# bitlayer-org/tap-stark

Measured on AMD Instinct MI355X. Metric: trace cells/sec (proofs/sec alongside), 2^20x64 BabyBear trace, higher is better.
Workload: dtype u32

## Files before the change

tap-stark_amd/csrc/kernels.hpp:

```cpp
#pragma once
#include <stdint.h>

#include "bb.hpp"
#include "context.hpp"

namespace ts {

struct ColMat {
    uint32_t* d = nullptr;
    uint64_t height = 0;
    uint32_t width = 0;
    uint64_t col_stride = 0;
};

void launch_build_twiddles(Context& ctx, uint32_t* W, uint32_t* Winv, unsigned log_size);
void launch_build_shift_tables(Context& ctx, uint32_t* lo, uint32_t* hi, uint32_t n_hi,
                               uint32_t n_cosets, uint32_t shift_mont, unsigned log_N,
                               unsigned log_blowup, uint32_t scale_mont);
const uint32_t* coset_scale_table(Context& ctx, unsigned log_n, unsigned log_blowup, uint32_t shift);
void launch_transpose_bitrev(Context& ctx, const uint32_t* src, uint32_t* dst, unsigned log_n,
                             uint32_t w, uint64_t dst_col_stride, uint32_t src_width = 0);
bool launch_transpose_bitrev_r16(Context& ctx, const uint32_t* src, uint32_t* dst, unsigned log_n, uint32_t w,
                                 uint64_t dst_col_stride, uint32_t src_width = 0);
void launch_transpose_plain(Context& ctx, const uint32_t* src, uint32_t* dst, uint64_t n, uint32_t w,
                            uint64_t dst_col_stride);
void launch_transpose_to_row_major(Context& ctx, const uint32_t* src, uint64_t col_stride,
                                   uint32_t* dst, uint64_t h, uint32_t w);
void coset_lde(Context& ctx, uint32_t* evals, uint64_t in_col_stride, uint32_t ncols, unsigned log_n,
               unsigned log_blowup, uint32_t shift, uint32_t* out, uint64_t out_col_stride,
               uint32_t beta0 = 0, uint32_t n_beta = 0, bool first_round_done = false,
               uint32_t* evals2 = nullptr, uint32_t shift2 = 0, uint32_t gw = 0);

constexpr int MAX_BATCH_MATS = 64;
struct LeafMats {
    const uint32_t* d[MAX_BATCH_MATS];
    uint64_t col_stride[MAX_BATCH_MATS];
    uint32_t width[MAX_BATCH_MATS];
    uint8_t row_shift[MAX_BATCH_MATS];
    uint32_t n_mats;
    uint32_t total_width;
    const uint32_t* const* cols;
};
void launch_leaf_hash(Context& ctx, const LeafMats& mats, uint64_t height, uint32_t* digests);
void launch_leaf_hash_ef_pairs(Context& ctx, const uint32_t* vec, uint64_t n_rows, uint32_t* digests);
struct DevChallenger;
bool launch_merkle_levels(Context& ctx, uint32_t* tree, unsigned log_leaves,
                          DevChallenger* ch = nullptr, uint32_t* root_out = nullptr,
                          Ef* beta_out = nullptr);
bool leaf_tree_enabled(unsigned log_leaves);
bool launch_commit_tree(Context& ctx, const LeafMats& mats, unsigned log_leaves, uint32_t* tree,
                        DevChallenger* ch = nullptr, uint32_t* root_out = nullptr, Ef* beta_out = nullptr);
bool launch_commit_tree_ef_pairs(Context& ctx, const uint32_t* vec, unsigned log_leaves, uint32_t* tree,
                                 DevChallenger* ch = nullptr, uint32_t* root_out = nullptr,
                                 Ef* beta_out = nullptr);
void launch_shard_top(Context& ctx, const uint32_t* subroots, uint32_t G, uint32_t* top,
                      DevChallenger* ch, uint32_t* root_out, Ef* beta_out);
void launch_merkle_one_level(Context& ctx, const uint32_t* children, uint32_t* parents,
                             uint64_t n_parents);
void launch_merkle_inject(Context& ctx, uint32_t* nodes, const uint32_t* inj, uint64_t n);
inline uint64_t merkle_level_offset(unsigned log_leaves, unsigned level) {
    uint64_t off = 0;
    for (unsigned l = 0; l < level; l++) off += (uint64_t)1 << (log_leaves - l);
    return off;
}
inline uint64_t merkle_total_digests(unsigned log_leaves) { return ((uint64_t)2 << log_leaves) - 1; }

struct AirProgram;
void launch_selectors(Context& ctx, unsigned log_n, unsigned log_qd, uint32_t* is_first,
                      uint32_t* is_last, uint32_t* is_transition, uint32_t shift = GENERATOR);
constexpr int MAX_QUOTIENT_CHUNKS = 64;
struct QuotOut {
    uint32_t* chunk[MAX_QUOTIENT_CHUNKS];
};
void launch_quotient(Context& ctx, const AirProgram& air, const ColMat& trace_lde, unsigned log_n,
                     unsigned log_qd, const uint32_t* d_consts_mont, const uint32_t* d_alpha_pows_mont,
                     const uint32_t* is_first, const uint32_t* is_last, const uint32_t* is_transition,
                     const QuotOut& out, uint64_t row_begin = 0, uint64_t row_end = 0,
                     uint32_t shift = GENERATOR);
void launch_chunk_mix(Context& ctx, uint32_t* const* d_chunk_ptrs, uint32_t qd, uint64_t rows, uint64_t col_stride,
                      const uint32_t* d_mix_mont);

void launch_check_constraints(Context& ctx, const AirProgram& air, const uint32_t* trace_row_major,
                              uint64_t n, const uint32_t* d_consts_mont,
                              unsigned long long* d_violation);

void launch_bary_weights(Context& ctx, unsigned log_n, const Ef* points_mont, uint32_t n_points,
                         Ef* out, uint32_t coset_gen = 0);
struct BaryPending {
    DevBuf<uint32_t> partial[2];
    uint32_t* out[2] = {nullptr, nullptr};
    uint32_t n_blocks[2] = {0, 0}, n_words[2] = {0, 0};
    uint32_t n = 0;
};
void launch_bary_dots(Context& ctx, const ColMat& m, unsigned log_n, const Ef* weights,
                      uint32_t n_points, Ef* out, BaryPending* pending = nullptr);
void launch_bary_finish(Context& ctx, BaryPending& pending);
struct ReduceArgs {
    Ef z_mont[2];
    Ef off_mont[2];
    Ef rys[2];
    uint32_t n_points;
    uint32_t accumulate;
};
void launch_reduce(Context& ctx, const ColMat& m, unsigned log_h, const uint32_t* d_alpha_pows_mont,
                   const ReduceArgs& args, Ef* ro);
struct FusedReduceArgs {
    Ef z_mont[2];
    Ef off_t[2];
    Ef k0, k1;
    const uint32_t* chunk_w;
    const uint32_t* chunk[MAX_QUOTIENT_CHUNKS];
    uint64_t chunk_stride;
    uint32_t n_chunks;
    uint64_t row0, rows;
};
void launch_reduce_fused(Context& ctx, const ColMat& trace, unsigned log_h,
                         const uint32_t* d_alpha_pows_mont, const FusedReduceArgs& args, Ef* ro);

void launch_fri_fold(Context& ctx, const Ef* in, uint64_t h, Ef beta_canonical, Ef* out,
                     uint32_t* next_digests);
void launch_fri_fold_dev(Context& ctx, const Ef* in, uint64_t h, const Ef* d_beta, Ef* out,
                         uint32_t* next_digests, uint64_t h_global = 0, uint64_t row0 = 0);
constexpr unsigned FRI_ROUND_MAX_LOG = 22;
void launch_fri_round(Context& ctx, const Ef* prev, const Ef* d_beta_prev, Ef* cur, uint64_t h,
                      uint32_t* tree, DevChallenger* ch, uint32_t* root_out, Ef* beta_out);
bool launch_fri_round_tall(Context& ctx, const Ef* prev, const Ef* d_beta_prev, Ef* cur, uint64_t h,
                           uint32_t* tree, DevChallenger* ch, uint32_t* root_out, Ef* beta_out,
                           uint64_t h_global = 0, uint64_t row0 = 0);
unsigned merkle_tree_max_log();
unsigned fri_round_max_log();
struct DevChallenger;
void launch_chal_round(Context& ctx, DevChallenger* ch, const uint32_t* root, uint32_t* root_out,
                       Ef* beta_out);
constexpr int FRI_TAIL_LOG = 10;
constexpr uint32_t FRI_POW_NONE = 0xffffffffu;
void launch_fri_tail(Context& ctx, const Ef* in, uint32_t L0, uint32_t blowup, DevChallenger* ch,
                     Ef* tail_vecs, uint32_t* tail_trees, uint32_t* roots_out, Ef* betas_out,
                     Ef* final_out, uint32_t pow_bits = 0, uint32_t* pow_out = nullptr,
                     const Ef* beta_in = nullptr);
void launch_vec_add(Context& ctx, Ef* acc, const Ef* other, uint64_t n);
void launch_gather_rows(Context& ctx, const LeafMats& mats, const uint32_t* d_indices,
                        uint32_t n_idx, unsigned index_shift, uint32_t* out);
void launch_gather_paths(Context& ctx, const uint32_t* tree, unsigned log_leaves,
                         const uint32_t* d_indices, uint32_t n_idx, unsigned index_shift,
                         uint32_t* out);
void launch_gather_ef_pairs(Context& ctx, const Ef* vec, const uint32_t* d_indices, uint32_t n_idx,
                            unsigned index_shift, uint32_t* out);
struct FriGatherDesc {
    const uint32_t* vec;
    const uint32_t* tree;
    uint32_t log_leaves;
    uint32_t shift;
    uint64_t out_vals;
    uint64_t out_path;
};
void launch_gather_fri(Context& ctx, const FriGatherDesc* d_descs, uint32_t n_rounds,
                       uint32_t max_log_leaves, const uint32_t* d_indices, uint32_t n_idx,
                       uint32_t* out);
struct RowGatherJob {
    LeafMats mats;
    uint32_t shift;
    uint32_t pad;
    uint64_t out;
};
void launch_gather_queries(Context& ctx, const RowGatherJob* d_rows, uint32_t n_rows, uint32_t max_row_width,
                           const FriGatherDesc* d_descs, uint32_t n_descs, uint32_t max_log_leaves,
                           const uint32_t* d_indices, uint32_t n_idx, uint32_t* out);

double alu_ceiling(Context& ctx, int kind);

void launch_trace_fibonacci(Context& ctx, uint32_t* out, uint32_t a, uint32_t b, uint64_t n);
void launch_trace_synth_mul(Context& ctx, uint32_t* out, uint64_t n, uint32_t width, uint64_t seed);
void launch_trace_synth_ext(Context& ctx, uint32_t* out, uint64_t n, uint32_t width, uint64_t seed);

}
```

tap-stark_amd/csrc/ntt_lde.hip:

```cpp
#include "kernels.hpp"

namespace ts {

constexpr int LOG_M = 12;
constexpr int NT_MID = 512;
constexpr int chunk_threads(int lm) { return lm == 14 ? 512 : 256; }
constexpr int TILE_ELEMS = 8192;

__device__ __forceinline__ uint32_t pad(uint32_t i) { return i + (i >> 5); }
constexpr int padded(int n) { return n + (n >> 5); }

template <int K, bool INV, bool TOP>
__device__ __forceinline__ void radix_butterflies(uint32_t (&v)[1 << K], unsigned s_base, unsigned u0,
                                                  uint32_t c, uint32_t hi,
                                                  const uint32_t* __restrict__ W) {
    constexpr int R = 1 << K;
    if (!INV) {
#pragma unroll
        for (int d = 0; d < K; d++) {
            const int half = R >> (d + 1);
            const uint32_t* __restrict__ wp = W + ((1u << (s_base + u0 + d)) + (c << (u0 + d)) + (hi << d));
#pragma unroll
            for (int q = 0; q < R; q++) {
                if ((q & half) == 0) {
                    const uint32_t a = red2p(v[q]);
                    uint32_t t = v[q + half];
                    if (TOP && (q >> (K - d)) == 0) t = red2p(t);
                    else t = mont_mul(t, wp[q >> (K - d)]);
                    v[q] = a + t;
                    v[q + half] = a - t + P;
                }
            }
        }
    } else {
#pragma unroll
        for (int d = K - 1; d >= 0; d--) {
            const int half = R >> (d + 1);
            const uint32_t* __restrict__ wp = W + ((1u << (s_base + u0 + d)) + (c << (u0 + d)) + (hi << d));
#pragma unroll
            for (int q = 0; q < R; q++) {
                if ((q & half) == 0) {
                    const uint32_t a = red2p(v[q]), b = red2p(v[q + half]);
                    v[q] = a + b;
                    uint32_t dlt = a - b + P;
                    if (!(TOP && (q >> (K - d)) == 0)) dlt = mont_mul_lazy(dlt, wp[q >> (K - d)]);
                    v[q + half] = dlt;
                }
            }
        }
    }
}

template <int K, bool INV, int LOG_DL, int NTH, bool TOP = false>
__device__ __forceinline__ void radix_round(uint32_t* s, unsigned log_total, unsigned u0,
                                            unsigned s_base, uint32_t c,
                                            const uint32_t* __restrict__ W) {
    constexpr int R = 1 << K;
    const unsigned log_dl = LOG_DL >= 0 ? (unsigned)LOG_DL : log_total - u0 - K;
    const uint32_t n_groups = 1u << (log_total - K);
    for (uint32_t g0 = threadIdx.x; g0 < n_groups; g0 += NTH) {
        uint32_t g = g0;
        if (LOG_DL == 4 && K < 5) {
            constexpr uint32_t B = 9 - K;
            const uint32_t x = ((g >> 4) ^ (g >> B)) & 1u;
            g ^= (x << 4) | (x << B);
        }
        const uint32_t lo = g & ((1u << log_dl) - 1);
        const uint32_t hi = g >> log_dl;
        const uint32_t base = (hi << (K + log_dl)) + lo;
        const uint32_t pbase = pad(base);
        uint32_t addr[R];
#pragma unroll
        for (int q = 0; q < R; q++) {
            if (LOG_DL >= 5)
                addr[q] = pbase + (uint32_t)q * ((1u << (LOG_DL >= 5 ? LOG_DL : 5)) +
                                                 (1u << (LOG_DL >= 5 ? LOG_DL - 5 : 0)));
            else if (LOG_DL == 4)
                addr[q] = pbase + 16u * (uint32_t)q + ((uint32_t)q >> 1);
            else if (LOG_DL == 0 && K == 4)
                addr[q] = pbase + (uint32_t)q;
            else
                addr[q] = pad(base + ((uint32_t)q << log_dl));
        }
        uint32_t v[R];
#pragma unroll
        for (int q = 0; q < R; q++) v[q] = s[addr[q]];
        radix_butterflies<K, INV, TOP>(v, s_base, u0, c, hi, W);
#pragma unroll
        for (int q = 0; q < R; q++) s[addr[q]] = v[q];
    }
    __syncthreads();
}

template <bool INV, int NTH>
__device__ __forceinline__ void radix_round_rt(int k, uint32_t* s, unsigned log_total, unsigned u0,
                                               unsigned s_base, uint32_t c,
                                               const uint32_t* __restrict__ W) {
    switch (k) {
        case 4: radix_round<4, INV, -1, NTH>(s, log_total, u0, s_base, c, W); break;
        case 3: radix_round<3, INV, -1, NTH>(s, log_total, u0, s_base, c, W); break;
        case 2: radix_round<2, INV, -1, NTH>(s, log_total, u0, s_base, c, W); break;
        default: radix_round<1, INV, -1, NTH>(s, log_total, u0, s_base, c, W); break;
    }
}

template <int NTH>
__device__ __forceinline__ void tile_forward_rt(uint32_t* s, unsigned log_len, unsigned log_T,
                                                unsigned s_base, uint32_t c,
                                                const uint32_t* __restrict__ W) {
    if (log_len == 0) return;
    const unsigned nr = (log_len + 3) / 4, q = log_len / nr, rem = log_len % nr;
    unsigned u = 0;
    for (unsigned r = 0; r < nr; r++) {
        const unsigned k = q + (r < rem ? 1u : 0u);
        radix_round_rt<false, NTH>((int)k, s, log_len + log_T, u, s_base, c, W);
        u += k;
    }
}
template <int NTH>
__device__ __forceinline__ void tile_inverse_rt(uint32_t* s, unsigned log_len, unsigned log_T,
                                                unsigned s_base, uint32_t c,
                                                const uint32_t* __restrict__ Winv) {
    if (log_len == 0) return;
    const unsigned nr = (log_len + 3) / 4, q = log_len / nr, rem = log_len % nr;
    unsigned u = log_len;
    for (int r = (int)nr - 1; r >= 0; r--) {
        const unsigned k = q + ((unsigned)r < rem ? 1u : 0u);
        u -= k;
        radix_round_rt<true, NTH>((int)k, s, log_len + log_T, u, s_base, c, Winv);
    }
}

template <int LM>
__device__ __forceinline__ void chunk_load(uint32_t* s, const uint32_t* __restrict__ g) {
    constexpr int NT = chunk_threads(LM);
    const uint4* g4 = reinterpret_cast<const uint4*>(g);
    uint4 v[(1 << LM) / 4 / NT];
#pragma unroll
    for (int k = 0; k < (1 << LM) / 4 / NT; k++) v[k] = g4[threadIdx.x + (uint32_t)k * NT];
#pragma unroll
    for (int k = 0; k < (1 << LM) / 4 / NT; k++) {
        const uint32_t i4 = threadIdx.x + (uint32_t)k * NT;
        const uint32_t a = 4 * i4 + (i4 >> 3);
        s[a] = v[k].x;
        s[a + 1] = v[k].y;
        s[a + 2] = v[k].z;
        s[a + 3] = v[k].w;
    }
    __syncthreads();
}
template <int LM, bool CANON>
__device__ __forceinline__ void chunk_store(const uint32_t* s, uint32_t* __restrict__ g) {
    constexpr int NT = chunk_threads(LM);
    uint4* g4 = reinterpret_cast<uint4*>(g);
#pragma unroll
    for (int k = 0; k < (1 << LM) / 4 / NT; k++) {
        const uint32_t i4 = threadIdx.x + (uint32_t)k * NT;
        const uint32_t a = 4 * i4 + (i4 >> 3);
        if (CANON)
            g4[i4] = make_uint4(red2p(s[a]), red2p(s[a + 1]), red2p(s[a + 2]), red2p(s[a + 3]));
        else
            g4[i4] = make_uint4(s[a], s[a + 1], s[a + 2], s[a + 3]);
    }
}

template <int LM, bool INV, bool SKIP_R16 = false>
__device__ __forceinline__ void chunk_rounds(uint32_t* s, unsigned sb, uint32_t c, const uint32_t* __restrict__ W) {
    constexpr int NT = chunk_threads(LM);
    constexpr int K0 = LM == 12 ? 4 : 5;
    constexpr int K1 = LM == 14 ? 5 : 4;
    static_assert(K0 + K1 + 4 == LM, "chunk plan");
    if (!INV) {
        radix_round<K0, false, LM - K0, NT>(s, LM, 0, sb, c, W);
        radix_round<K1, false, 4, NT>(s, LM, K0, sb, c, W);
        radix_round<4, false, 0, NT>(s, LM, K0 + K1, sb, c, W);
    } else {
        if (!SKIP_R16) radix_round<4, true, 0, NT>(s, LM, K0 + K1, sb, c, W);
        radix_round<K1, true, 4, NT>(s, LM, K0, sb, c, W);
        radix_round<K0, true, LM - K0, NT>(s, LM, 0, sb, c, W);
    }
}

template <int LM, bool SKIP_R16 = false>
__global__ void __launch_bounds__(chunk_threads(LM))
k_intt_contig(uint32_t* __restrict__ data, uint64_t col_stride, unsigned log_n,
              const uint32_t* __restrict__ Winv, uint32_t* __restrict__ data2, uint32_t gw) {
    __shared__ uint32_t s[padded(1 << LM)];
    const uint32_t c = blockIdx.x;
    uint32_t* col = blockIdx.y < gw ? data + (uint64_t)blockIdx.y * col_stride
                                    : data2 + (uint64_t)(blockIdx.y - gw) * col_stride;
    uint32_t* g = col + ((uint64_t)c << LM);
    chunk_load<LM>(s, g);
    chunk_rounds<LM, true, SKIP_R16>(s, log_n - LM, c, Winv);
    chunk_store<LM, false>(s, g);
}

__global__ void __launch_bounds__(256)
k_transpose_bitrev_r16(const uint32_t* __restrict__ src, uint32_t* __restrict__ dst, unsigned log_n,
                       uint32_t w, uint64_t dst_col_stride, uint32_t src_width,
                       const uint32_t* __restrict__ Winv) {
    __shared__ uint32_t tile[64][65];
    const uint32_t p0 = blockIdx.x << 6;
    const uint32_t c0 = blockIdx.y * 64;
    const uint32_t tx = threadIdx.x & 63, ty = threadIdx.x >> 6;
    const uint32_t rb = bitrev32(p0, log_n);
    const uint64_t row_step = (uint64_t)src_width << (log_n - 6);
    uint32_t v[16];
    if (c0 + tx < w) {
        const uint32_t* sp = src + (uint64_t)rb * src_width + c0 + tx;
#pragma unroll
        for (int q = 0; q < 16; q++) v[q] = sp[(uint64_t)(__brev(16 * ty + (uint32_t)q) >> 26) * row_step];
    } else {
#pragma unroll
        for (int q = 0; q < 16; q++) v[q] = 0;
    }
    radix_butterflies<4, true, false>(v, log_n - 4, 0, 0, (p0 >> 4) + ty, Winv);
#pragma unroll
    for (int q = 0; q < 16; q++) tile[16 * ty + q][tx] = v[q];
    __syncthreads();
    uint32_t t[16];
#pragma unroll
    for (int k = 0; k < 16; k++) t[k] = tile[tx][ty + 4 * k];
    uint32_t* dp = dst + (uint64_t)(c0 + ty) * dst_col_stride + p0 + tx;
#pragma unroll
    for (int k = 0; k < 16; k++)
        if (c0 + ty + 4 * k < w) dp[(uint64_t)(4 * k) * dst_col_stride] = t[k];
}

template <int LM, int CPW = 1>
__global__ void __launch_bounds__(chunk_threads(LM), CPW > 1 ? 4 : 1)
k_lde_fwd_contig(uint32_t* __restrict__ out, uint64_t out_col_stride, unsigned log_n,
                 const uint32_t* __restrict__ W) {
    __shared__ uint32_t s[padded(1 << LM)];
    constexpr int NT = chunk_threads(LM);
    constexpr int NV = (1 << LM) / 4 / NT;
    const uint32_t beta = blockIdx.z;
    uint32_t* col = out + (uint64_t)blockIdx.y * out_col_stride + ((uint64_t)beta << log_n);
    if constexpr (CPW == 1) {
        const uint32_t c = blockIdx.x;
        uint32_t* o = col + ((uint64_t)c << LM);
        chunk_load<LM>(s, o);
        chunk_rounds<LM, false>(s, log_n - LM, c, W);
        chunk_store<LM, true>(s, o);
    } else {
        const uint32_t c0 = blockIdx.x * CPW;
        uint4 v[NV];
        {
            const uint4* g4 = reinterpret_cast<const uint4*>(col + ((uint64_t)c0 << LM));
#pragma unroll
            for (int k = 0; k < NV; k++) v[k] = g4[threadIdx.x + (uint32_t)k * NT];
        }
#pragma unroll 1
        for (int i = 0; i < CPW; i++) {
            const uint32_t c = c0 + i;
#pragma unroll
            for (int k = 0; k < NV; k++) {
                const uint32_t i4 = threadIdx.x + (uint32_t)k * NT;
                const uint32_t a = 4 * i4 + (i4 >> 3);
                s[a] = v[k].x;
                s[a + 1] = v[k].y;
                s[a + 2] = v[k].z;
                s[a + 3] = v[k].w;
            }
            __syncthreads();
            if (i + 1 < CPW) {
                const uint4* g4 = reinterpret_cast<const uint4*>(col + ((uint64_t)(c + 1) << LM));
#pragma unroll
                for (int k = 0; k < NV; k++) v[k] = g4[threadIdx.x + (uint32_t)k * NT];
            }
            chunk_rounds<LM, false>(s, log_n - LM, c, W);
            chunk_store<LM, true>(s, col + ((uint64_t)c << LM));
            __syncthreads();
        }
    }
}

template <int PLAN, int TILE = TILE_ELEMS, int NTM = NT_MID, int LM = LOG_M>
__global__ void __launch_bounds__(NTM)
k_lde_mid(const uint32_t* __restrict__ evals, uint64_t in_col_stride, uint32_t* __restrict__ out,
          uint64_t out_col_stride, unsigned log_n, unsigned log_len, unsigned log_T,
          unsigned row_shift, unsigned beta0, unsigned n_cosets, const uint32_t* __restrict__ W,
          const uint32_t* __restrict__ Winv, const uint32_t* __restrict__ scale_a,
          const uint32_t* __restrict__ evals2, const uint32_t* __restrict__ scale_b, uint32_t gw) {
    __shared__ uint32_t s[padded(TILE)];
    constexpr int PER_THREAD = TILE / NTM;
    if (PLAN == 1) {
        log_len = 8;
        log_T = 5;
    }
    const bool remap = PLAN == 0 && log_T < 5 && gridDim.x >= 8;
    uint32_t bx = remap ? (blockIdx.x & 7) * (gridDim.x >> 3) + (blockIdx.x >> 3) : blockIdx.x;
    uint32_t col_id = blockIdx.y;
    if constexpr (PLAN == 1) {
        const uint32_t ncols = gridDim.x >> (LM - 5);
        bx = (blockIdx.x & 31) + 32 * (blockIdx.x / (32 * ncols));
        col_id = (blockIdx.x >> 5) % ncols;
    }
    const uint32_t j2_0 = bx << log_T;
    const uint32_t* g = (col_id < gw ? evals + (uint64_t)col_id * in_col_stride
                                     : evals2 + (uint64_t)(col_id - gw) * in_col_stride) + j2_0;
    const uint32_t* __restrict__ scale = col_id < gw ? scale_a : scale_b;
    const uint32_t total = 1u << (log_len + log_T);
    const uint32_t tmask = (1u << log_T) - 1;
    if constexpr (PLAN == 1) {
        uint32_t t[PER_THREAD];
#pragma unroll
        for (int k = 0; k < PER_THREAD; k++) {
            const uint32_t i = threadIdx.x + (uint32_t)k * NTM;
            t[k] = g[((uint64_t)(i >> log_T) << row_shift) + (i & tmask)];
        }
#pragma unroll
        for (int k = 0; k < PER_THREAD; k++) s[pad(threadIdx.x + (uint32_t)k * NTM)] = t[k];
    } else {
        for (uint32_t i = threadIdx.x; i < total; i += NTM)
            s[pad(i)] = g[((uint64_t)(i >> log_T) << row_shift) + (i & tmask)];
    }
    __syncthreads();
    if (PLAN == 1) {
        radix_round<4, true, 5, NTM>(s, 13, 4, 0, 0, Winv);
    } else {
        tile_inverse_rt<NTM>(s, log_len, log_T, 0, 0, Winv);
    }
    uint32_t coef[PER_THREAD];
#pragma unroll
    for (int k = 0; k < PER_THREAD; k++) {
        const uint32_t i = threadIdx.x + (uint32_t)k * NTM;
        coef[k] = i < total ? s[pad(i)] : 0u;
    }
    constexpr int GP = PER_THREAD / 16;
    if constexpr (PLAN == 1) {
#pragma unroll
        for (int j = 0; j < GP; j++) {
            uint32_t v[16];
#pragma unroll
            for (int q = 0; q < 16; q++) v[q] = coef[j + GP * q];
            radix_butterflies<4, true, true>(v, 0, 0, 0, 0, Winv);
#pragma unroll
            for (int q = 0; q < 16; q++) coef[j + GP * q] = v[q];
        }
    }
    constexpr bool PREFETCH = PLAN == 1;
    uint32_t scv[PREFETCH ? 16 : 1];
    const uint32_t* scp = nullptr;
    if constexpr (PREFETCH) {
        const uint32_t i0 = threadIdx.x;
        scp = scale + ((uint64_t)(i0 >> 5) << LM) + (i0 & 31) + j2_0;
#pragma unroll
        for (int q = 0; q < 16; q++)
            scv[q] = (scp + ((uint64_t)beta0 << log_n))[(uint64_t)q * (NTM >> 5) << LM];
    }
    for (uint32_t bl = 0; bl < n_cosets; bl++) {
        const uint32_t beta = beta0 + bl;
        const uint32_t* sc = scale + ((uint64_t)beta << log_n);
        __syncthreads();
        if constexpr (PLAN == 1) {
#pragma unroll
            for (int j = 0; j < GP; j++) {
                uint32_t v[16];
#pragma unroll
                for (int q = 0; q < 16; q++) v[q] = mont_mul_lazy(coef[j + GP * q], scv[q]);
                if (bl + 1 < n_cosets) {
                    const uint32_t* nx = scp + ((uint64_t)(beta + 1) << log_n);
#pragma unroll
                    for (int q = 0; q < 16; q++) scv[q] = nx[(uint64_t)q * (NTM >> 5) << LM];
                }
                radix_butterflies<4, false, true>(v, 0, 0, 0, 0, W);
#pragma unroll
                for (int q = 0; q < 16; q++) s[pad(threadIdx.x + (uint32_t)(j + GP * q) * NTM)] = v[q];
            }
            __syncthreads();
            uint32_t* og = out + (uint64_t)col_id * out_col_stride + ((uint64_t)bl << log_n) + j2_0;
            radix_round<4, false, 5, NTM>(s, 13, 4, 0, 0, W);
            uint32_t t[PER_THREAD];
#pragma unroll
            for (int k = 0; k < PER_THREAD; k++) t[k] = s[pad(threadIdx.x + (uint32_t)k * NTM)];
            uint32_t* ot = og + ((uint64_t)(threadIdx.x >> 5) << LM) + (threadIdx.x & 31);
#pragma unroll
            for (int k = 0; k < PER_THREAD; k++) ot[(uint64_t)k * (NTM >> 5) << LM] = t[k];
            continue;
        } else {
#pragma unroll
            for (int k = 0; k < PER_THREAD; k++) {
                const uint32_t i = threadIdx.x + (uint32_t)k * NTM;
                if (i < total) {
                    const uint32_t kk = ((i >> log_T) << row_shift) + (i & tmask) + j2_0;
                    s[pad(i)] = mont_mul_lazy(coef[k], sc[kk]);
                }
            }
            __syncthreads();
            tile_forward_rt<NTM>(s, log_len, log_T, 0, 0, W);
        }
        uint32_t* o = out + (uint64_t)col_id * out_col_stride + ((uint64_t)bl << log_n) + j2_0;
        if (row_shift != 0) {
            for (uint32_t i = threadIdx.x; i < total; i += NTM)
                o[((uint64_t)(i >> log_T) << row_shift) + (i & tmask)] = s[pad(i)];
        } else {
            for (uint32_t i = threadIdx.x; i < total; i += NTM)
                o[((uint64_t)(i >> log_T) << row_shift) + (i & tmask)] = red2p(s[pad(i)]);
        }
    }
}

static unsigned lde_chunk_log(unsigned log_n) {
    return (log_n == 21 || log_n == 22) ? log_n - 8 : (unsigned)LOG_M;
}

bool launch_transpose_bitrev_r16(Context& ctx, const uint32_t* src, uint32_t* dst, unsigned log_n, uint32_t w,
                                 uint64_t dst_col_stride, uint32_t src_width) {
    if (w == 0 || log_n <= lde_chunk_log(log_n)) return false;
    ctx.ensure_twiddles(log_n);
    TS_LAUNCH(ctx, k_transpose_bitrev_r16, dim3(1u << (log_n - 6), (w + 63) / 64), dim3(256), 0, src, dst, log_n, w,
              dst_col_stride, src_width ? src_width : w, (const uint32_t*)ctx.d_twiddle_inv);
    TS_HIP(hipGetLastError());
    return true;
}

void coset_lde(Context& ctx, uint32_t* evals, uint64_t in_col_stride, uint32_t ncols, unsigned log_n,
               unsigned log_blowup, uint32_t shift, uint32_t* out, uint64_t out_col_stride,
               uint32_t beta0, uint32_t n_beta, bool first_round_done, uint32_t* evals2, uint32_t shift2,
               uint32_t gw) {
    if (ncols == 0) return;
    TS_REQUIRE(evals2 == nullptr || (gw >= 1 && gw < ncols && shift2 != 0), TS_ERR_INVALID,
               "coset_lde: second matrix needs its first column and its shift");
    if (evals2 == nullptr) gw = 0xffffffffu;
    TS_REQUIRE(log_n + log_blowup <= 27, TS_ERR_INVALID, "coset_lde: log_n + log_blowup > 27");
    TS_REQUIRE(ncols >= 1 && ncols <= 65535, TS_ERR_INVALID, "coset_lde: bad column count");
    const unsigned LM = lde_chunk_log(log_n);
    TS_REQUIRE(!first_round_done || log_n > LM, TS_ERR_INVARIANT, "coset_lde: no contiguous inverse pass at this size");
    const bool two_pass = log_n > LM;
    const unsigned sA = two_pass ? log_n - LM : 0;
    TS_REQUIRE(sA <= 14, TS_ERR_INVALID, "coset_lde: log_n > 26");
    ctx.ensure_twiddles(log_n == 0 ? 1 : log_n);
    const uint32_t* W = ctx.d_twiddle_fwd;
    const uint32_t* Winv = ctx.d_twiddle_inv;
    unsigned log_T = 0;
    if (two_pass && sA <= 13)
        while ((1u << (sA + log_T + 1)) <= (unsigned)TILE_ELEMS && log_T < 6) log_T++;

    const uint32_t n_cosets = 1u << log_blowup;
    if (n_beta == 0) n_beta = n_cosets - beta0;
    TS_REQUIRE(beta0 < n_cosets && n_beta <= n_cosets - beta0, TS_ERR_INVALID, "coset_lde: coset range");
    const uint32_t* scale = coset_scale_table(ctx, log_n, log_blowup, shift);
    const uint32_t* scale2 = evals2 ? coset_scale_table(ctx, log_n, log_blowup, shift2) : nullptr;

    if (two_pass) {
        TS_REQUIRE(in_col_stride % 4 == 0 && out_col_stride % 4 == 0, TS_ERR_INVALID,
                   "coset_lde: column strides must be multiples of 4 elements");
        if (ctx.lde_pass_mask & 1u) {
            StageTimer t(&ctx, "lde: inverse NTT, contiguous stages");
            const dim3 g(1u << sA, ncols);
#define TS_INTT(LMV)                                                                                          \
    do {                                                                                                      \
        if (first_round_done)                                                                                 \
            TS_LAUNCH(ctx, (k_intt_contig<LMV, true>), g, dim3(chunk_threads(LMV)), 0, evals, in_col_stride, log_n, \
                      Winv, evals2, gw);                                                                      \
        else                                                                                                  \
            TS_LAUNCH(ctx, k_intt_contig<LMV>, g, dim3(chunk_threads(LMV)), 0, evals, in_col_stride, log_n, Winv, \
                      evals2, gw);                                                                            \
    } while (0)
            if (LM == 12) TS_INTT(12);
            else if (LM == 13) TS_INTT(13);
            else TS_INTT(14);
#undef TS_INTT
        }
        StageTimer t_rest(&ctx, "lde: strided pass + forward NTT of the owned cosets");
        const dim3 grid(1u << (LM - log_T), ncols);
        const dim3 grid1((1u << (LM - log_T)) * ncols);
#define TS_MID_ARGS                                                                            \
    (const uint32_t*)evals, in_col_stride, out, out_col_stride, log_n, sA, log_T, (unsigned)LM, \
        beta0, n_beta, W, Winv, scale, (const uint32_t*)evals2, scale2, gw
        if (!(ctx.lde_pass_mask & 2u)) {
        } else if (sA == 14)
            TS_LAUNCH(ctx, (k_lde_mid<0, 16384>), grid, dim3(NT_MID), 0, TS_MID_ARGS);
        else if (sA == 8 && log_T == 5 && LM == 12)
            TS_LAUNCH(ctx, k_lde_mid<1>, grid1, dim3(NT_MID), 0, TS_MID_ARGS);
        else if (sA == 8 && log_T == 5 && LM == 13)
            TS_LAUNCH(ctx, (k_lde_mid<1, 8192, 512, 13>), grid1, dim3(NT_MID), 0, TS_MID_ARGS);
        else if (sA == 8 && log_T == 5 && LM == 14)
            TS_LAUNCH(ctx, (k_lde_mid<1, 8192, 512, 14>), grid1, dim3(NT_MID), 0, TS_MID_ARGS);
        else
            TS_LAUNCH(ctx, k_lde_mid<0>, grid, dim3(NT_MID), 0, TS_MID_ARGS);
        const dim3 gf(1u << sA, ncols, n_beta);
        if (!(ctx.lde_pass_mask & 4u)) {
        } else if (LM == 12)
            TS_LAUNCH(ctx, k_lde_fwd_contig<12>, gf, dim3(chunk_threads(12)), 0, out, out_col_stride, log_n, W);
        else if (LM == 13)
            TS_LAUNCH(ctx, k_lde_fwd_contig<13>, gf, dim3(chunk_threads(13)), 0, out, out_col_stride, log_n, W);
        else
            TS_LAUNCH(ctx, (k_lde_fwd_contig<14, 4>), dim3(gf.x / 4, gf.y, gf.z), dim3(chunk_threads(14)), 0, out,
                      out_col_stride, log_n, W);
    } else {
        TS_LAUNCH(ctx, k_lde_mid<0>, dim3(1, ncols), dim3(NT_MID), 0, (const uint32_t*)evals,
                  in_col_stride, out, out_col_stride, log_n, log_n, 0u, 0u, beta0, n_beta, W, Winv, scale,
                  (const uint32_t*)evals2, scale2, gw);
    }
    TS_HIP(hipGetLastError());
}

}
```

tap-stark_amd/csrc/prover_common.cpp:

```cpp
#include <stdlib.h>
#include <string.h>

#include <optional>

#include "prover_internal.hpp"

namespace ts {

void h2d(Context& ctx, void* dst, const void* src, size_t bytes) {
    if (!bytes) return;
    const void* from = bytes <= (1u << 20) ? ctx.stage(src, bytes) : src;
    TS_HIP(hipMemcpyAsync(dst, from, bytes, hipMemcpyHostToDevice, ctx.stream));
}
void d2h_sync(Context& ctx, void* dst, const void* src, size_t bytes) {
    if (bytes) TS_HIP(hipMemcpyAsync(dst, src, bytes, hipMemcpyDeviceToHost, ctx.stream));
    ctx.sync();
}

unsigned log2_strict(uint64_t n) {
    unsigned k = 0;
    while ((1ull << k) < n) k++;
    TS_REQUIRE((1ull << k) == n, TS_ERR_INVALID, "height must be a power of two");
    return k;
}

Ef efc_mul(Ef a, Ef b) { return ef_mul(a, ef_to_mont(b)); }
Ef efc_mul_base(Ef a, uint32_t b) { return ef_mul_base(a, to_mont(b)); }
Ef efc_pow(Ef a, uint64_t e) { return ef_from_mont(ef_pow(ef_to_mont(a), e)); }

std::vector<const uint32_t*> column_pointers(const std::vector<ColMat>& ldes, uint64_t height) {
    std::vector<const uint32_t*> cols;
    for (auto& cm : ldes)
        if (!height || cm.height == height)
            for (uint32_t c = 0; c < cm.width; c++) cols.push_back(cm.d + (uint64_t)c * cm.col_stride);
    return cols;
}

bool columns_as_one_matrix(const std::vector<ColMat>& ldes, uint64_t height, uint32_t max_width, ColMat& one) {
    const ColMat* first = nullptr;
    uint32_t wsum = 0;
    for (auto& cm : ldes)
        if (cm.height == height) {
            if (!first) first = &cm;
            if (cm.col_stride != first->col_stride || cm.d != first->d + (uint64_t)wsum * first->col_stride)
                return false;
            wsum += cm.width;
        }
    if (!wsum || (max_width && wsum > max_width)) return false;
    one = *first;
    one.width = wsum;
    return true;
}

LeafMats PcsData::leaf_mats() const {
    LeafMats lm;
    memset(&lm, 0, sizeof lm);
    lm.n_mats = (uint32_t)ldes.size();
    for (size_t i = 0; i < ldes.size(); i++) {
        lm.d[i] = ldes[i].d;
        lm.col_stride[i] = ldes[i].col_stride;
        lm.width[i] = ldes[i].width;
        lm.row_shift[i] = (uint8_t)(log_height - log2_strict(ldes[i].height));
        lm.total_width += ldes[i].width;
    }
    lm.cols = col_table_uploaded ? col_table.p : nullptr;
    return lm;
}

LeafMats PcsData::leaf_mats_with_table(Context& ctx) {
    if (!col_table_uploaded) {
        const std::vector<const uint32_t*> cols = column_pointers(ldes);
        col_table = DevBuf<const uint32_t*>(&ctx, cols.size());
        h2d(ctx, col_table.p, cols.data(), cols.size() * sizeof(const uint32_t*));
        col_table_uploaded = true;
    }
    return leaf_mats();
}

void lde_stage(Context& ctx, const FriConfig& fri, std::vector<DeviceMatrix>& evals,
               const std::vector<uint32_t>& domain_shifts, uint32_t beta0, uint32_t n_beta, bool allow_pair,
               PcsData& data) {
    TS_REQUIRE(!evals.empty() && evals.size() <= (size_t)MAX_BATCH_MATS, TS_ERR_INVALID,
               "commit: between 1 and MAX_BATCH_MATS (64) matrices per batch");
    TS_REQUIRE(evals.size() == domain_shifts.size(), TS_ERR_INVALID, "commit: one domain per matrix");
    uint64_t max_n = 0;
    bool same_height = true;
    size_t total_w = 0;
    for (size_t i = 0; i < evals.size(); i++) {
        const DeviceMatrix& m = evals[i];
        TS_REQUIRE(m.width >= 1 && m.buf.p, TS_ERR_INVALID, "commit: empty matrix");
        TS_REQUIRE(domain_shifts[i] != 0 && domain_shifts[i] < P, TS_ERR_INVALID, "bad domain shift");
        log2_strict(m.height);
        max_n = std::max(max_n, m.height);
        same_height = same_height && m.height == evals[0].height;
        total_w += m.width;
    }
    TS_REQUIRE(same_height || !n_beta, TS_ERR_INVALID, "sharded commit: matrices of one height expected");
    const unsigned log_N = log2_strict(max_n) + fri.log_blowup;
    TS_REQUIRE(log_N <= 27, TS_ERR_INVALID, "commit: LDE larger than the two-adic subgroup");
    ctx.ensure_twiddles(std::max(1u, log_N));
    auto lde_rows = [&](uint64_t n) { return n_beta ? (uint64_t)n_beta * n : n << fri.log_blowup; };
    data.log_height = log2_strict(lde_rows(max_n));
    auto push_lde = [&](uint32_t* d, uint64_t rows, uint32_t width) {
        ColMat cm;
        cm.d = d;
        cm.height = rows;
        cm.width = width;
        cm.col_stride = rows;
        data.ldes.push_back(cm);
    };

    StageTimer t(&ctx, "coset_lde");
    const bool batched = same_height && evals.size() > 1;
    DevBuf<uint32_t> batch;
    if (batched) batch = DevBuf<uint32_t>(&ctx, total_w * lde_rows(evals[0].height));
    size_t batch_col = 0;
    static const bool pair_knob = [] { const char* e = getenv("TS_LDE_PAIR"); return !e || atoi(e) != 0; }();
    if (allow_pair && pair_knob && batched && evals.size() == 2 && evals[0].width == evals[1].width &&
        evals[0].layout == DeviceMatrix::COL_MAJOR_BITREV && evals[1].layout == DeviceMatrix::COL_MAJOR_BITREV) {
        const uint64_t n = evals[0].height, rows = lde_rows(n);
        const uint32_t w = evals[0].width;
        coset_lde(ctx, evals[0].buf.p, n, 2 * w, log2_strict(n), fri.log_blowup,
                  mul(GENERATOR, inv_canon(domain_shifts[0])), batch.p, rows, beta0, n_beta, false, evals[1].buf.p,
                  mul(GENERATOR, inv_canon(domain_shifts[1])), w);
        for (size_t i = 0; i < 2; i++) {
            push_lde(batch.p + i * (size_t)w * rows, rows, w);
            evals[i].buf.reset();
        }
        data.lde_storage.push_back(std::move(batch));
        return;
    }
    for (size_t i = 0; i < evals.size(); i++) {
        DeviceMatrix& m = evals[i];
        const uint64_t n = m.height, rows = lde_rows(n);
        const unsigned log_n = log2_strict(n);
        DevBuf<uint32_t> colmajor;
        uint32_t* ev = m.buf.p;
        bool r16 = false;
        if (m.layout == DeviceMatrix::ROW_MAJOR) {
            std::optional<StageTimer> tt;
            if (n_beta) tt.emplace(&ctx, "lde: transpose (every column on every rank)");
            colmajor = DevBuf<uint32_t>(&ctx, (size_t)m.width * n);
            r16 = launch_transpose_bitrev_r16(ctx, m.buf.p, colmajor.p, log_n, m.width, n);
            if (!r16) launch_transpose_bitrev(ctx, m.buf.p, colmajor.p, log_n, m.width, n);
            ev = colmajor.p;
        }
        DevBuf<uint32_t> own;
        uint32_t* lde;
        if (batched) {
            lde = batch.p + batch_col * rows;
            batch_col += m.width;
        } else {
            own = DevBuf<uint32_t>(&ctx, (size_t)m.width * rows);
            lde = own.p;
        }
        coset_lde(ctx, ev, n, m.width, log_n, fri.log_blowup, mul(GENERATOR, inv_canon(domain_shifts[i])), lde,
                  rows, beta0, n_beta, r16);
        push_lde(lde, rows, m.width);
        if (!batched) data.lde_storage.push_back(std::move(own));
        m.buf.reset();
    }
    if (batched) data.lde_storage.push_back(std::move(batch));
}

Statement check_statement(const FriConfig& fri, const AirProgram& air, uint32_t trace_width, uint64_t degree,
                          size_t n_public_values) {
    TS_REQUIRE(trace_width == air.width, TS_ERR_INVALID, "prove: trace width != AIR width");
    TS_REQUIRE(n_public_values == air.n_public, TS_ERR_INVALID, "prove: wrong number of public values");
    Statement s;
    s.log_degree = log2_strict(degree);
    s.lqd = air.log_quotient_degree;
    s.qd = 1u << s.lqd;
    s.log_N = s.log_degree + fri.log_blowup;
    s.w = air.width;
    TS_REQUIRE(s.lqd <= fri.log_blowup, TS_ERR_INVARIANT,
               "quotient domain larger than the committed LDE (log_quotient_degree > log_blowup)");
    return s;
}

std::vector<uint32_t> alpha_powers_mont(Ef alpha, size_t count) {
    std::vector<uint32_t> pw(4 * count);
    const Ef am = ef_to_mont(alpha);
    Ef cur = ef_one_mont();
    for (size_t i = 0; i < count; i++) {
        memcpy(&pw[4 * i], cur.c, 16);
        cur = ef_mul(cur, am);
    }
    return pw;
}

Ef bary_scale(Ef point, uint32_t coset_gen, uint64_t n) {
    Ef un = efc_pow(efc_mul_base(point, inv_canon(coset_gen)), n);
    un.c[0] = sub(un.c[0], 1);
    return efc_mul_base(un, inv_canon((uint32_t)(n % P)));
}

std::vector<uint32_t> chunk_domain_shifts(uint32_t base_shift, unsigned log_degree, unsigned lqd) {
    std::vector<uint32_t> shifts(1u << lqd);
    const uint32_t gq = two_adic_generator(log_degree + lqd);
    for (uint32_t c = 0; c < shifts.size(); c++) shifts[c] = mul(base_shift, pow_canon(gq, c));
    return shifts;
}

size_t ProofWriter::words_per_query(const std::vector<Batch>& batches, const std::vector<unsigned>& round_depths,
                                    size_t n_pass_through) {
    size_t n = 1 + 5 * n_pass_through;
    for (auto& b : batches) {
        n += 1 + b.mats->size() + 1 + 8 * (size_t)b.depth;
        for (auto& m : *b.mats) n += m.width;
    }
    for (unsigned d : round_depths) n += 8 + 1 + 8 * (size_t)d;
    return n;
}

void ProofWriter::header(uint32_t version, unsigned log_degree, uint32_t width, uint32_t qd, uint32_t num_queries) {
    out_.push_back(TSPF_MAGIC);
    out_.push_back(version);
    out_.push_back(log_degree);
    out_.push_back(width);
    out_.push_back(qd);
    if (version >= 2) out_.push_back(num_queries);
}

void ProofWriter::opened_values(const std::vector<Ef>& values) {
    for (auto& e : values) words(e.c, 4);
}

void ProofWriter::path(std::initializer_list<Path> parts) {
    for (auto& part : parts) {
        if (!swap_) words(part.digests, 8 * part.depth);
        else for (size_t k = 0; k < 8 * part.depth; k++) out_.push_back(__builtin_bswap32(part.digests[k]));
    }
}

void ProofWriter::pass_through_value(unsigned log_height, const uint32_t value[4]) {
    out_.push_back(log_height);
    words(value, 4);
}

void ProofWriter::batch_opening(const std::vector<ColMat>& mats, const uint32_t* row, unsigned depth,
                                std::initializer_list<Path> parts) {
    out_.push_back((uint32_t)mats.size());
    for (auto& m : mats) {
        out_.push_back(m.width);
        words(row, m.width);
        row += m.width;
    }
    out_.push_back(depth);
    path(parts);
}

void ProofWriter::round_opening(const uint32_t values[8], unsigned depth, std::initializer_list<Path> parts) {
    words(values, 8);
    out_.push_back(depth);
    path(parts);
}

void ProofWriter::finish(Ef final_poly, uint32_t pow_witness) {
    words(final_poly.c, 4);
    out_.push_back(pow_witness);
}

}
```

Measured before the change: 24.80 billion.

## Fuse row-major transpose with contiguous inverse NTT and skip the trivially known coset

```diff
diff --git a/tap-stark_amd/csrc/kernels.hpp b/tap-stark_amd/csrc/kernels.hpp
--- a/tap-stark_amd/csrc/kernels.hpp
+++ b/tap-stark_amd/csrc/kernels.hpp
@@ -22,13 +22,16 @@
                              uint32_t w, uint64_t dst_col_stride, uint32_t src_width = 0);
 bool launch_transpose_bitrev_r16(Context& ctx, const uint32_t* src, uint32_t* dst, unsigned log_n, uint32_t w,
                                  uint64_t dst_col_stride, uint32_t src_width = 0);
+bool launch_intt_contig_rm(Context& ctx, const uint32_t* src, uint32_t* dst, unsigned log_n, uint32_t w,
+                           uint64_t dst_col_stride, uint32_t src_width = 0);
+enum InverseDone { INV_NONE = 0, INV_R16 = 1, INV_CONTIG = 2 };
 void launch_transpose_plain(Context& ctx, const uint32_t* src, uint32_t* dst, uint64_t n, uint32_t w,
                             uint64_t dst_col_stride);
 void launch_transpose_to_row_major(Context& ctx, const uint32_t* src, uint64_t col_stride,
                                    uint32_t* dst, uint64_t h, uint32_t w);
 void coset_lde(Context& ctx, uint32_t* evals, uint64_t in_col_stride, uint32_t ncols, unsigned log_n,
                unsigned log_blowup, uint32_t shift, uint32_t* out, uint64_t out_col_stride,
-               uint32_t beta0 = 0, uint32_t n_beta = 0, bool first_round_done = false,
+               uint32_t beta0 = 0, uint32_t n_beta = 0, InverseDone inverse_done = INV_NONE,
                uint32_t* evals2 = nullptr, uint32_t shift2 = 0, uint32_t gw = 0);
 
 constexpr int MAX_BATCH_MATS = 64;
diff --git a/tap-stark_amd/csrc/ntt_lde.hip b/tap-stark_amd/csrc/ntt_lde.hip
--- a/tap-stark_amd/csrc/ntt_lde.hip
+++ b/tap-stark_amd/csrc/ntt_lde.hip
@@ -9,6 +9,13 @@
 
 __device__ __forceinline__ uint32_t pad(uint32_t i) { return i + (i >> 5); }
 constexpr int padded(int n) { return n + (n >> 5); }
+
+constexpr uint32_t NO_BLOCK = 0xffffffffu;
+struct KnownBlock {
+    uint32_t* out;
+    uint64_t out_col_stride;
+    uint32_t a, b;
+};
 
 template <int K, bool INV, bool TOP>
 __device__ __forceinline__ void radix_butterflies(uint32_t (&v)[1 << K], unsigned s_base, unsigned u0,
@@ -51,14 +58,14 @@
     }
 }
 
-template <int K, bool INV, int LOG_DL, int NTH, bool TOP = false>
+template <int K, bool INV, int LOG_DL, int NTH, bool TOP = false, bool SYNC = true>
 __device__ __forceinline__ void radix_round(uint32_t* s, unsigned log_total, unsigned u0,
                                             unsigned s_base, uint32_t c,
-                                            const uint32_t* __restrict__ W) {
+                                            const uint32_t* __restrict__ W, const uint32_t tid = threadIdx.x) {
     constexpr int R = 1 << K;
     const unsigned log_dl = LOG_DL >= 0 ? (unsigned)LOG_DL : log_total - u0 - K;
     const uint32_t n_groups = 1u << (log_total - K);
-    for (uint32_t g0 = threadIdx.x; g0 < n_groups; g0 += NTH) {
+    for (uint32_t g0 = tid; g0 < n_groups; g0 += NTH) {
         uint32_t g = g0;
         if (LOG_DL == 4 && K < 5) {
             constexpr uint32_t B = 9 - K;
@@ -89,7 +96,7 @@
 #pragma unroll
         for (int q = 0; q < R; q++) s[addr[q]] = v[q];
     }
-    __syncthreads();
+    if (SYNC) __syncthreads();
 }
 
 template <bool INV, int NTH>
@@ -132,12 +139,19 @@
 }
 
 template <int LM>
-__device__ __forceinline__ void chunk_load(uint32_t* s, const uint32_t* __restrict__ g) {
+__device__ __forceinline__ void chunk_load(uint32_t* s, const uint32_t* __restrict__ g,
+                                           uint32_t* __restrict__ copy = nullptr) {
     constexpr int NT = chunk_threads(LM);
     const uint4* g4 = reinterpret_cast<const uint4*>(g);
     uint4 v[(1 << LM) / 4 / NT];
 #pragma unroll
     for (int k = 0; k < (1 << LM) / 4 / NT; k++) v[k] = g4[threadIdx.x + (uint32_t)k * NT];
+    if (copy) {
+        uint4* c4 = reinterpret_cast<uint4*>(copy);
+#pragma unroll
+        for (int k = 0; k < (1 << LM) / 4 / NT; k++)
+            c4[threadIdx.x + (uint32_t)k * NT] = make_uint4(red2p(v[k].x), red2p(v[k].y), red2p(v[k].z), red2p(v[k].w));
+    }
 #pragma unroll
     for (int k = 0; k < (1 << LM) / 4 / NT; k++) {
         const uint32_t i4 = threadIdx.x + (uint32_t)k * NT;
@@ -184,15 +198,89 @@
 template <int LM, bool SKIP_R16 = false>
 __global__ void __launch_bounds__(chunk_threads(LM))
 k_intt_contig(uint32_t* __restrict__ data, uint64_t col_stride, unsigned log_n,
-              const uint32_t* __restrict__ Winv, uint32_t* __restrict__ data2, uint32_t gw) {
+              const uint32_t* __restrict__ Winv, uint32_t* __restrict__ data2, uint32_t gw,
+              KnownBlock kb) {
     __shared__ uint32_t s[padded(1 << LM)];
     const uint32_t c = blockIdx.x;
     uint32_t* col = blockIdx.y < gw ? data + (uint64_t)blockIdx.y * col_stride
                                     : data2 + (uint64_t)(blockIdx.y - gw) * col_stride;
     uint32_t* g = col + ((uint64_t)c << LM);
-    chunk_load<LM>(s, g);
+    uint32_t* copy = nullptr;
+    if (!SKIP_R16) {
+        const uint32_t known = blockIdx.y < gw ? kb.a : kb.b;
+        if (known != NO_BLOCK)
+            copy = kb.out + (uint64_t)blockIdx.y * kb.out_col_stride + ((uint64_t)known << log_n) + ((uint64_t)c << LM);
+    }
+    chunk_load<LM>(s, g, copy);
     chunk_rounds<LM, true, SKIP_R16>(s, log_n - LM, c, Winv);
     chunk_store<LM, false>(s, g);
+}
+
+template <int LM, int CW, bool XCD_ORDER>
+__global__ void __launch_bounds__(CW * 128, 4)
+k_intt_contig_rm(const uint32_t* __restrict__ src, uint32_t* __restrict__ dst, unsigned log_n, uint32_t w,
+                 uint64_t dst_col_stride, uint32_t src_width, const uint32_t* __restrict__ Winv) {
+    static_assert(LM == 12 && (CW == 4 || CW == 8), "fused row-major inverse pass: plan");
+    constexpr int NT = CW * 128;
+    constexpr int IMG = padded(1 << LM);
+    __shared__ uint32_t s[CW * IMG];
+    const unsigned sA = log_n - LM;
+    const uint32_t ncg = w / CW;
+    uint32_t c, cg;
+    if (XCD_ORDER) {
+        const uint32_t m = blockIdx.x >> 3;
+        cg = m % ncg;
+        c = ((m / ncg) << 3) + (blockIdx.x & 7);
+    } else {
+        c = blockIdx.x / ncg;
+        cg = blockIdx.x % ncg;
+    }
+    const uint32_t c0 = cg * CW;
+    {
+        constexpr int NV = (1 << LM) * (CW / 4) / NT;
+        const uint32_t* sp = src + (uint64_t)bitrev32(c, sA) * src_width + c0;
+        uint4 v[NV];
+        uint32_t pos[NV];
+#pragma unroll
+        for (int m = 0; m < NV; m++) {
+            const uint32_t e = threadIdx.x + (uint32_t)m * NT;
+            const uint32_t half = CW == 8 ? (e >> 5) & 1u : 0u;
+            const uint32_t k = ((e & 31u) << 7) | (CW == 8 ? e >> 6 : e >> 5);
+            v[m] = *reinterpret_cast<const uint4*>(sp + (((uint64_t)k << sA) * src_width + 4 * half));
+            pos[m] = 4 * half * IMG + pad(__brev(k) >> (32 - LM));
+        }
+#pragma unroll
+        for (int m = 0; m < NV; m++) {
+            s[pos[m]] = v[m].x;
+            s[pos[m] + IMG] = v[m].y;
+            s[pos[m] + 2 * IMG] = v[m].z;
+            s[pos[m] + 3 * IMG] = v[m].w;
+        }
+    }
+    __syncthreads();
+    const uint32_t tx = threadIdx.x & 255u;
+    uint32_t* s0 = s + (threadIdx.x >> 8) * 2 * IMG;
+    const unsigned sb = log_n - LM;
+    radix_round<4, true, 0, 256, false, false>(s0, LM, 8, sb, c, Winv, tx);
+    radix_round<4, true, 0, 256, false, false>(s0 + IMG, LM, 8, sb, c, Winv, tx);
+    __syncthreads();
+    radix_round<4, true, 4, 256, false, false>(s0, LM, 4, sb, c, Winv, tx);
+    radix_round<4, true, 4, 256, false, false>(s0 + IMG, LM, 4, sb, c, Winv, tx);
+    __syncthreads();
+    radix_round<4, true, LM - 4, 256, false, false>(s0, LM, 0, sb, c, Winv, tx);
+    radix_round<4, true, LM - 4, 256, false, false>(s0 + IMG, LM, 0, sb, c, Winv, tx);
+    __syncthreads();
+    {
+        constexpr int NV = (1 << LM) / 4 * CW / NT;
+        uint32_t* dp = dst + (uint64_t)c0 * dst_col_stride + ((uint64_t)c << LM);
+#pragma unroll
+        for (int m = 0; m < NV; m++) {
+            const uint32_t e = threadIdx.x + (uint32_t)m * NT;
+            const uint32_t j = e >> (LM - 2), i4 = e & ((1u << (LM - 2)) - 1);
+            const uint32_t a = j * IMG + 4 * i4 + (i4 >> 3);
+            reinterpret_cast<uint4*>(dp + (uint64_t)j * dst_col_stride)[i4] = make_uint4(s[a], s[a + 1], s[a + 2], s[a + 3]);
+        }
+    }
 }
 
 __global__ void __launch_bounds__(256)
@@ -230,11 +318,15 @@
 template <int LM, int CPW = 1>
 __global__ void __launch_bounds__(chunk_threads(LM), CPW > 1 ? 4 : 1)
 k_lde_fwd_contig(uint32_t* __restrict__ out, uint64_t out_col_stride, unsigned log_n,
-                 const uint32_t* __restrict__ W) {
+                 const uint32_t* __restrict__ W, uint32_t known_a, uint32_t known_b, uint32_t gw,
+                 uint32_t compact) {
     __shared__ uint32_t s[padded(1 << LM)];
     constexpr int NT = chunk_threads(LM);
     constexpr int NV = (1 << LM) / 4 / NT;
-    const uint32_t beta = blockIdx.z;
+    uint32_t beta = blockIdx.z;
+    const uint32_t known = blockIdx.y < gw ? known_a : known_b;
+    if (compact) beta += beta >= known ? 1u : 0u;
+    else if (beta == known) return;
     uint32_t* col = out + (uint64_t)blockIdx.y * out_col_stride + ((uint64_t)beta << log_n);
     if constexpr (CPW == 1) {
         const uint32_t c = blockIdx.x;
@@ -281,7 +373,8 @@
           uint64_t out_col_stride, unsigned log_n, unsigned log_len, unsigned log_T,
           unsigned row_shift, unsigned beta0, unsigned n_cosets, const uint32_t* __restrict__ W,
           const uint32_t* __restrict__ Winv, const uint32_t* __restrict__ scale_a,
-          const uint32_t* __restrict__ evals2, const uint32_t* __restrict__ scale_b, uint32_t gw) {
+          const uint32_t* __restrict__ evals2, const uint32_t* __restrict__ scale_b, uint32_t gw,
+          uint32_t known_a, uint32_t known_b) {
     __shared__ uint32_t s[padded(TILE)];
     constexpr int PER_THREAD = TILE / NTM;
     if (PLAN == 1) {
@@ -300,6 +393,7 @@
     const uint32_t* g = (col_id < gw ? evals + (uint64_t)col_id * in_col_stride
                                      : evals2 + (uint64_t)(col_id - gw) * in_col_stride) + j2_0;
     const uint32_t* __restrict__ scale = col_id < gw ? scale_a : scale_b;
+    const uint32_t known = col_id < gw ? known_a : known_b;
     const uint32_t total = 1u << (log_len + log_T);
     const uint32_t tmask = (1u << log_T) - 1;
     if constexpr (PLAN == 1) {
@@ -342,14 +436,18 @@
     constexpr bool PREFETCH = PLAN == 1;
     uint32_t scv[PREFETCH ? 16 : 1];
     const uint32_t* scp = nullptr;
+    const uint32_t bl_first = known == 0 ? 1u : 0u;
     if constexpr (PREFETCH) {
         const uint32_t i0 = threadIdx.x;
         scp = scale + ((uint64_t)(i0 >> 5) << LM) + (i0 & 31) + j2_0;
-#pragma unroll
-        for (int q = 0; q < 16; q++)
-            scv[q] = (scp + ((uint64_t)beta0 << log_n))[(uint64_t)q * (NTM >> 5) << LM];
-    }
-    for (uint32_t bl = 0; bl < n_cosets; bl++) {
+        if (bl_first < n_cosets) {
+#pragma unroll
+            for (int q = 0; q < 16; q++)
+                scv[q] = (scp + ((uint64_t)(beta0 + bl_first) << log_n))[(uint64_t)q * (NTM >> 5) << LM];
+        }
+    }
+    for (uint32_t bl = bl_first, bl_next; bl < n_cosets; bl = bl_next) {
+        bl_next = bl + 1 == known ? bl + 2 : bl + 1;
         const uint32_t beta = beta0 + bl;
         const uint32_t* sc = scale + ((uint64_t)beta << log_n);
         __syncthreads();
@@ -359,8 +457,8 @@
                 uint32_t v[16];
 #pragma unroll
                 for (int q = 0; q < 16; q++) v[q] = mont_mul_lazy(coef[j + GP * q], scv[q]);
-                if (bl + 1 < n_cosets) {
-                    const uint32_t* nx = scp + ((uint64_t)(beta + 1) << log_n);
+                if (bl_next < n_cosets) {
+                    const uint32_t* nx = scp + ((uint64_t)(beta0 + bl_next) << log_n);
 #pragma unroll
                     for (int q = 0; q < 16; q++) scv[q] = nx[(uint64_t)q * (NTM >> 5) << LM];
                 }
@@ -415,9 +513,42 @@
     return true;
 }
 
+bool launch_intt_contig_rm(Context& ctx, const uint32_t* src, uint32_t* dst, unsigned log_n, uint32_t w,
+                           uint64_t dst_col_stride, uint32_t src_width) {
+    static const int knob = [] { const char* e = getenv("TS_INTT_FUSED"); return e ? atoi(e) : 8; }();
+    if (src_width == 0) src_width = w;
+    if (knob == 0 || w == 0 || log_n <= (unsigned)LOG_M || lde_chunk_log(log_n) != (unsigned)LOG_M) return false;
+    const uint32_t cw = knob == 4 ? 4 : 8;
+    if (w % cw != 0 || src_width % 4 != 0 || dst_col_stride % 4 != 0 || ((uintptr_t)src | (uintptr_t)dst) % 16 != 0)
+        return false;
+    ctx.ensure_twiddles(log_n);
+    const unsigned sA = log_n - LOG_M;
+    const dim3 grid((w / cw) << sA);
+#define TS_RM(CW, XO)                                                                                         \
+    TS_LAUNCH(ctx, (k_intt_contig_rm<12, CW, XO>), grid, dim3(CW * 128), 0, src, dst, log_n, w, dst_col_stride, \
+              src_width, (const uint32_t*)ctx.d_twiddle_inv)
+    if (cw == 8) {
+        if (sA >= 3) TS_RM(8, true);
+        else TS_RM(8, false);
+    } else {
+        if (sA >= 3) TS_RM(4, true);
+        else TS_RM(4, false);
+    }
+#undef TS_RM
+    TS_HIP(hipGetLastError());
+    return true;
+}
+
+static uint32_t known_block(uint32_t shift, unsigned log_n, unsigned log_blowup, uint32_t beta0, uint32_t n_beta) {
+    const uint32_t wN = two_adic_generator(log_n + log_blowup);
+    for (uint32_t bl = 0; bl < n_beta; bl++)
+        if (mul(shift, pow_canon(wN, bitrev32(beta0 + bl, log_blowup))) == 1) return bl;
+    return NO_BLOCK;
+}
+
 void coset_lde(Context& ctx, uint32_t* evals, uint64_t in_col_stride, uint32_t ncols, unsigned log_n,
                unsigned log_blowup, uint32_t shift, uint32_t* out, uint64_t out_col_stride,
-               uint32_t beta0, uint32_t n_beta, bool first_round_done, uint32_t* evals2, uint32_t shift2,
+               uint32_t beta0, uint32_t n_beta, InverseDone inverse_done, uint32_t* evals2, uint32_t shift2,
                uint32_t gw) {
     if (ncols == 0) return;
     TS_REQUIRE(evals2 == nullptr || (gw >= 1 && gw < ncols && shift2 != 0), TS_ERR_INVALID,
@@ -426,7 +557,7 @@
     TS_REQUIRE(log_n + log_blowup <= 27, TS_ERR_INVALID, "coset_lde: log_n + log_blowup > 27");
     TS_REQUIRE(ncols >= 1 && ncols <= 65535, TS_ERR_INVALID, "coset_lde: bad column count");
     const unsigned LM = lde_chunk_log(log_n);
-    TS_REQUIRE(!first_round_done || log_n > LM, TS_ERR_INVARIANT, "coset_lde: no contiguous inverse pass at this size");
+    TS_REQUIRE(inverse_done == INV_NONE || log_n > LM, TS_ERR_INVARIANT, "coset_lde: no contiguous inverse pass at this size");
     const bool two_pass = log_n > LM;
     const unsigned sA = two_pass ? log_n - LM : 0;
     TS_REQUIRE(sA <= 14, TS_ERR_INVALID, "coset_lde: log_n > 26");
@@ -443,20 +574,29 @@
     const uint32_t* scale = coset_scale_table(ctx, log_n, log_blowup, shift);
     const uint32_t* scale2 = evals2 ? coset_scale_table(ctx, log_n, log_blowup, shift2) : nullptr;
 
+    static const bool known_knob = [] { const char* e = getenv("TS_LDE_KNOWN"); return !e || atoi(e) != 0; }();
+    KnownBlock kb{out, out_col_stride, NO_BLOCK, NO_BLOCK};
+    if (known_knob && two_pass && inverse_done == INV_NONE && log_blowup >= 1 && beta0 == 0 && n_beta == n_cosets &&
+        ctx.lde_pass_mask == 7u) {
+        kb.a = known_block(shift, log_n, log_blowup, beta0, n_beta);
+        if (evals2) kb.b = known_block(shift2, log_n, log_blowup, beta0, n_beta);
+    }
+    const bool compact = kb.a != NO_BLOCK && (!evals2 || kb.b != NO_BLOCK);
+
     if (two_pass) {
         TS_REQUIRE(in_col_stride % 4 == 0 && out_col_stride % 4 == 0, TS_ERR_INVALID,
                    "coset_lde: column strides must be multiples of 4 elements");
-        if (ctx.lde_pass_mask & 1u) {
+        if ((ctx.lde_pass_mask & 1u) && inverse_done != INV_CONTIG) {
             StageTimer t(&ctx, "lde: inverse NTT, contiguous stages");
             const dim3 g(1u << sA, ncols);
 #define TS_INTT(LMV)                                                                                          \
     do {                                                                                                      \
-        if (first_round_done)                                                                                 \
+        if (inverse_done == INV_R16)                                                                          \
             TS_LAUNCH(ctx, (k_intt_contig<LMV, true>), g, dim3(chunk_threads(LMV)), 0, evals, in_col_stride, log_n, \
-                      Winv, evals2, gw);                                                                      \
+                      Winv, evals2, gw, kb);                                                                  \
         else                                                                                                  \
             TS_LAUNCH(ctx, k_intt_contig<LMV>, g, dim3(chunk_threads(LMV)), 0, evals, in_col_stride, log_n, Winv, \
-                      evals2, gw);                                                                            \
+                      evals2, gw, kb);                                                                        \
     } while (0)
             if (LM == 12) TS_INTT(12);
             else if (LM == 13) TS_INTT(13);
@@ -468,7 +608,7 @@
         const dim3 grid1((1u << (LM - log_T)) * ncols);
 #define TS_MID_ARGS                                                                            \
     (const uint32_t*)evals, in_col_stride, out, out_col_stride, log_n, sA, log_T, (unsigned)LM, \
-        beta0, n_beta, W, Winv, scale, (const uint32_t*)evals2, scale2, gw
+        beta0, n_beta, W, Winv, scale, (const uint32_t*)evals2, scale2, gw, kb.a, kb.b
         if (!(ctx.lde_pass_mask & 2u)) {
         } else if (sA == 14)
             TS_LAUNCH(ctx, (k_lde_mid<0, 16384>), grid, dim3(NT_MID), 0, TS_MID_ARGS);
@@ -480,19 +620,21 @@
             TS_LAUNCH(ctx, (k_lde_mid<1, 8192, 512, 14>), grid1, dim3(NT_MID), 0, TS_MID_ARGS);
         else
             TS_LAUNCH(ctx, k_lde_mid<0>, grid, dim3(NT_MID), 0, TS_MID_ARGS);
-        const dim3 gf(1u << sA, ncols, n_beta);
-        if (!(ctx.lde_pass_mask & 4u)) {
+        const dim3 gf(1u << sA, ncols, compact ? n_beta - 1 : n_beta);
+#define TS_FWD_ARGS out, out_col_stride, log_n, W, kb.a, kb.b, gw, (uint32_t)compact
+        if (!(ctx.lde_pass_mask & 4u) || gf.z == 0) {
         } else if (LM == 12)
-            TS_LAUNCH(ctx, k_lde_fwd_contig<12>, gf, dim3(chunk_threads(12)), 0, out, out_col_stride, log_n, W);
+            TS_LAUNCH(ctx, k_lde_fwd_contig<12>, gf, dim3(chunk_threads(12)), 0, TS_FWD_ARGS);
         else if (LM == 13)
-            TS_LAUNCH(ctx, k_lde_fwd_contig<13>, gf, dim3(chunk_threads(13)), 0, out, out_col_stride, log_n, W);
+            TS_LAUNCH(ctx, k_lde_fwd_contig<13>, gf, dim3(chunk_threads(13)), 0, TS_FWD_ARGS);
         else
-            TS_LAUNCH(ctx, (k_lde_fwd_contig<14, 4>), dim3(gf.x / 4, gf.y, gf.z), dim3(chunk_threads(14)), 0, out,
-                      out_col_stride, log_n, W);
+            TS_LAUNCH(ctx, (k_lde_fwd_contig<14, 4>), dim3(gf.x / 4, gf.y, gf.z), dim3(chunk_threads(14)), 0,
+                      TS_FWD_ARGS);
+#undef TS_FWD_ARGS
     } else {
         TS_LAUNCH(ctx, k_lde_mid<0>, dim3(1, ncols), dim3(NT_MID), 0, (const uint32_t*)evals,
                   in_col_stride, out, out_col_stride, log_n, log_n, 0u, 0u, beta0, n_beta, W, Winv, scale,
-                  (const uint32_t*)evals2, scale2, gw);
+                  (const uint32_t*)evals2, scale2, gw, NO_BLOCK, NO_BLOCK);
     }
     TS_HIP(hipGetLastError());
 }
diff --git a/tap-stark_amd/csrc/prover_common.cpp b/tap-stark_amd/csrc/prover_common.cpp
--- a/tap-stark_amd/csrc/prover_common.cpp
+++ b/tap-stark_amd/csrc/prover_common.cpp
@@ -121,7 +121,7 @@
         const uint64_t n = evals[0].height, rows = lde_rows(n);
         const uint32_t w = evals[0].width;
         coset_lde(ctx, evals[0].buf.p, n, 2 * w, log2_strict(n), fri.log_blowup,
-                  mul(GENERATOR, inv_canon(domain_shifts[0])), batch.p, rows, beta0, n_beta, false, evals[1].buf.p,
+                  mul(GENERATOR, inv_canon(domain_shifts[0])), batch.p, rows, beta0, n_beta, INV_NONE, evals[1].buf.p,
                   mul(GENERATOR, inv_canon(domain_shifts[1])), w);
         for (size_t i = 0; i < 2; i++) {
             push_lde(batch.p + i * (size_t)w * rows, rows, w);
@@ -136,13 +136,14 @@
         const unsigned log_n = log2_strict(n);
         DevBuf<uint32_t> colmajor;
         uint32_t* ev = m.buf.p;
-        bool r16 = false;
+        InverseDone inv = INV_NONE;
         if (m.layout == DeviceMatrix::ROW_MAJOR) {
             std::optional<StageTimer> tt;
             if (n_beta) tt.emplace(&ctx, "lde: transpose (every column on every rank)");
             colmajor = DevBuf<uint32_t>(&ctx, (size_t)m.width * n);
-            r16 = launch_transpose_bitrev_r16(ctx, m.buf.p, colmajor.p, log_n, m.width, n);
-            if (!r16) launch_transpose_bitrev(ctx, m.buf.p, colmajor.p, log_n, m.width, n);
+            if (launch_intt_contig_rm(ctx, m.buf.p, colmajor.p, log_n, m.width, n)) inv = INV_CONTIG;
+            else if (launch_transpose_bitrev_r16(ctx, m.buf.p, colmajor.p, log_n, m.width, n)) inv = INV_R16;
+            else launch_transpose_bitrev(ctx, m.buf.p, colmajor.p, log_n, m.width, n);
             ev = colmajor.p;
         }
         DevBuf<uint32_t> own;
@@ -155,7 +156,7 @@
             lde = own.p;
         }
         coset_lde(ctx, ev, n, m.width, log_n, fri.log_blowup, mul(GENERATOR, inv_canon(domain_shifts[i])), lde,
-                  rows, beta0, n_beta, r16);
+                  rows, beta0, n_beta, inv);
         push_lde(lde, rows, m.width);
         if (!batched) data.lde_storage.push_back(std::move(own));
         m.buf.reset();
```

New measurement: 24.32 billion. 0.981x the previous value.
